# isaac-chandler/cuda-raytracer

Measured on AMD Instinct MI355X. Metric: Mrays/s (live ray segments/s, teapot), higher is better.
Workload: dtype f32

## Files before the change

### cuda-raytracer_amd/csrc/rt_device.h

```cpp
#pragma once
#include <hip/hip_runtime.h>
#include <stdint.h>

#pragma clang fp contract(off)

#define RT_HD __host__ __device__ __forceinline__

namespace rtd {

struct V3 { float x, y, z; };

RT_HD V3 v3(float x, float y, float z) { return {x, y, z}; }
RT_HD V3 operator+(V3 a, V3 b) { return {a.x + b.x, a.y + b.y, a.z + b.z}; }
RT_HD V3 operator-(V3 a, V3 b) { return {a.x - b.x, a.y - b.y, a.z - b.z}; }
RT_HD V3 operator*(V3 a, V3 b) { return {a.x * b.x, a.y * b.y, a.z * b.z}; }
RT_HD V3 operator*(float s, V3 v) { return {s * v.x, s * v.y, s * v.z}; }
RT_HD V3 operator-(V3 v) { return {-v.x, -v.y, -v.z}; }
RT_HD float dot(V3 a, V3 b) { return a.x * b.x + a.y * b.y + a.z * b.z; }
RT_HD V3 cross(V3 a, V3 b) {
    return {a.y * b.z - a.z * b.y, a.z * b.x - a.x * b.z, a.x * b.y - a.y * b.x};
}
RT_HD float magsq(V3 v) { return v.x * v.x + v.y * v.y + v.z * v.z; }
RT_HD V3 normalise(V3 v) { return (1.0f / sqrtf(magsq(v))) * v; }
RT_HD float clamp01(float x) { return fmaxf(fminf(x, 1.0f), 0.0f); }
// ... 64 lines not shown
    const V3 a = (o - min_coord) * inv_dim;
    const V3 b = 0.5f * (d + v3(1, 1, 1));
    return (quant_bit(a.z) << 5) | (quant_bit(a.y) << 4) | (quant_bit(a.x) << 3) |
           (quant_bit(b.z) << 2) | (quant_bit(b.y) << 1) | quant_bit(b.x);
}

RT_HD bool slab(float lx, float ly, float lz, float hx, float hy, float hz, V3 o, float ix, float iy, float iz,
                float tmax, float &tmin) {
    tmin = 0.0f;
    float t1 = (lx - o.x) * ix, t2 = (hx - o.x) * ix;
    tmin = fminf(fmaxf(t1, tmin), fmaxf(t2, tmin));
    tmax = fmaxf(fminf(t1, tmax), fminf(t2, tmax));
    t1 = (ly - o.y) * iy; t2 = (hy - o.y) * iy;
    tmin = fminf(fmaxf(t1, tmin), fmaxf(t2, tmin));
    tmax = fmaxf(fminf(t1, tmax), fminf(t2, tmax));
    t1 = (lz - o.z) * iz; t2 = (hz - o.z) * iz;
    tmin = fminf(fmaxf(t1, tmin), fmaxf(t2, tmin));
    tmax = fmaxf(fminf(t1, tmax), fminf(t2, tmax));
    return tmin <= tmax;
}

RT_HD bool ray_triangle(V3 o, V3 d, V3 p1, V3 e1, V3 e2, float closest, float &t) {
    const V3 h = cross(d, e2);
    const float a = dot(h, e1);
    if (a == 0) return false;
    const float f = 1 / a;
    const V3 s = o - p1;
    const float u = dot(s, h) * f;
    if (u < 0 || u > 1) return false;
    const V3 q = cross(s, e1);
    const float v = dot(d, q) * f;
    if (v < 0 || u + v > 1) return false;
    t = dot(e2, q) * f;
    return !(t < kEps || t >= closest);
}

RT_HD bool ray_sphere(V3 o, V3 d, V3 c, float radius, float closest, float &t) {
    const V3 off = c - o;
    const float mhb = dot(off, d);
    const float qc = magsq(off) - radius * radius;
    const float qd = mhb * mhb - qc;
    if (qd < 0) return false;
    const float hs = sqrtf(qd);
    t = mhb - hs;
    if (t < closest && !(t < kEps)) return true;
    t = mhb + hs;
    return t < closest && !(t < kEps);
}

RT_HD V3 sky_color(const float *env, int env_w, int env_h, V3 dir) {
    const float dx = (float)((double)dir.x * -0.386527 + (double)dir.z * 0.922278);
    const float dy = (float)((double)dir.x * -0.922278 + (double)dir.z * -0.386527);
    const float dz = dir.y;
    const float x = fabsf(dx), y = fabsf(dy), z = fabsf(dz);
    const float r = sqrtf(1 - fminf(z, 1.0f));
    const float a = fmaxf(x, y);
    float b = fminf(x, y);
    b = a == 0 ? 0 : b / a;
    float phi = (float)((2 / 3.14159265358979323846) * (double)rt_atan01(b));
    if (x < y) phi = 1 - phi;
    float v = phi * r;
    float u = r - v;
    if (dz < 0) {
        const float old_v = v;
        v = 1 - u;
        u = 1 - old_v;
    }
    u = copysignf(u, dx);
    v = copysignf(v, dy);
    const float cu = (u + 1) * 0.5f, cv = (v + 1) * 0.5f;
    const int tx = (int)((double)(clamp01(cu) * (env_w - 1)) + 0.5);
    const int ty = (int)((double)(clamp01(cv) * (env_h - 1)) + 0.5);
    const float *e = env + (size_t)(ty * env_h + tx) * 3;
    return v3(e[0], e[1], e[2]);
}

struct Mat { V3 diffuse; float metal; V3 spec; float rough; V3 emit; float ior; };

RT_HD Mat load_mat(const float4 *m) {
    const float4 a = m[0], b = m[1], c = m[2];
    return {v3(a.x, a.y, a.z), a.w, v3(b.x, b.y, b.z), b.w, v3(c.x, c.y, c.z), c.w};
}

RT_HD void scatter(V3 d, V3 normal, const Mat &m, Rng &rng, V3 &T, V3 &C, V3 &nd) {
    C = C + m.emit * T;
    const bool front = dot(normal, d) < 0;
    if (!front) normal = -normal;
    const V3 rough = normalise(normal + m.rough * random_on_sphere(rng));
    const float cos_theta = dot(rough, d);
    if (m.ior == 0) {
        if (random01(rng) <= m.metal) {
            T = T * m.spec;
            nd = d - (2 * cos_theta) * rough;
        } else {
            T = T * m.diffuse;
            nd = normalise(normal + random_on_sphere(rng));
        }
    } else {
        float ior = m.ior;
        float inv_ior = 1 / ior;
        if (front) { const float tmp = inv_ior; inv_ior = ior; ior = tmp; }
        const float sin2 = 1 - cos_theta * cos_theta;
        float r0 = (1 - ior) / (1 + ior);
        r0 *= r0;
        const float cs = 1 + cos_theta;
        const float refl = r0 + (1 - r0) * cs * cs * cs * cs * cs;
        if (sin2 > inv_ior * inv_ior || random01(rng) < refl) {
            T = T * m.spec;
            nd = d - (2 * cos_theta) * rough;
        } else {
            T = T * m.diffuse;
            const V3 perp = ior * (d - cos_theta * rough);
            const V3 par = (-sqrtf(1 - magsq(perp))) * rough;
            nd = normalise(par + perp);
        }
    }
}

}
```

### cuda-raytracer_amd/csrc/rt_render.hip

```cpp
#include "rt_common.h"

#include <algorithm>
#include <chrono>
#include <cstdio>
#include <cstdlib>
#include <cstring>
#include <string>
#include <thread>
#include <vector>

#include <rccl/rccl.h>

#pragma clang fp contract(off)

int rtamd_render_multi(const rt_scene *scene, const rt_opts *opts, float *fb_out, rt_stats *stats);

using namespace rtamd;

namespace {

#ifndef RT_INFLIGHT
#define RT_INFLIGHT 20
#endif
#ifndef RT_TRACE_OCC
// ... 169 lines not shown
            const bool empty = sp == 0;
            sp = empty ? 0 : sp - 1;
            uint2 e = col[min(sp, kStackLds) * kBlock];
            asm volatile("" : "+v"(e.x), "+v"(e.y));
            if (__builtin_expect(__ballot(sp >= kStackLds) != 0, 0)) {
                if (sp >= kStackLds) {
                    e.x = overflow[(sp - kStackLds) * lanes + gl];
                    e.y = overflow[dist_half + (sp - kStackLds) * lanes + gl];
                }
            }
            const bool take = !empty && !(__uint_as_float(e.y) >= closest);
            slot = empty ? -2 - slot : slot;
            ref = take ? e.x : ref;
            if (COUNT) pn += take ? 1u : 0u;
            const bool leaf = take && (ref & kLeaf);
            if (__builtin_expect(leaf && (ref & kBigLeaf), 0)) {
                leaf_range(S, ref, ti, te);
            } else {
                ti = leaf ? (int)(ref & 0xFFFFFFu) : ti;
                te = leaf ? ti + (int)((ref >> 24) & 0x3Fu) : te;
            }
            need = !empty && (!take || (leaf && ti == te));
        }
    };
    const bool root_internal = !(S.root_ref & kLeaf);
    float4 ra{0, 0, 0, 0}, rb{0, 0, 0, 0}, rc{0, 0, 0, 0};
    uint2 rk{0, 0};
    if (root_internal) {
        const float4 *rr = S.nodes + (size_t)S.root_ref * 4;
        const float4 x0 = rr[0], x1 = rr[1], x2 = rr[2];
        const uint2 k = *reinterpret_cast<const uint2 *>(rr + 3);
#define RT_U(v) __int_as_float(__builtin_amdgcn_readfirstlane(__float_as_int(v)))
        ra = make_float4(RT_U(x0.x), RT_U(x0.y), RT_U(x0.z), RT_U(x0.w));
        rb = make_float4(RT_U(x1.x), RT_U(x1.y), RT_U(x1.z), RT_U(x1.w));
        rc = make_float4(RT_U(x2.x), RT_U(x2.y), RT_U(x2.z), RT_U(x2.w));
#undef RT_U
        rk = make_uint2(__builtin_amdgcn_readfirstlane(k.x), __builtin_amdgcn_readfirstlane(k.y));
    }
    while (true) {
        unsigned long long idle = __ballot(slot < 0);
        if (!exhausted && __popcll(idle) >= (FIRST ? kRefillFirst : kRefill)) {
            PROF(6, 1);
            if (slot <= -2) {
                hits[-2 - slot] = make_float2(closest, __int_as_float(index));
                slot = -1;
            }
            bool fresh = false;
            do {
                bool got = false;
                while (idle && !exhausted) {
                    if (q_next >= q_end) {
                        const uint32_t seg_lo = (uint32_t)(((uint64_t)L * shard) / kQueues);
                        const uint32_t seg_hi = (uint32_t)(((uint64_t)L * (shard + 1)) / kQueues);
                        uint32_t c = 0;
                        if (lane_id() == 0) c = atomicAdd(queue + shard * kQueueStride, chunk);
                        c = __builtin_amdgcn_readfirstlane(__shfl(c, 0)) + seg_lo;
                        if (c >= seg_hi) {
                            shard = (shard + 1) % kQueues;
                            if (++tried == kQueues) exhausted = true;
                            continue;
                        }
                        q_next = c;
                        q_end = min(c + chunk, seg_hi);
                    }
                    const uint32_t avail = q_end - q_next;
                    const uint32_t r = rank_below(idle);
                    const bool take = slot < 0 && r < avail;
                    const unsigned long long took = __ballot(take);
                    if (take) { slot = (int)(q_next + r); fresh = true; got = true; }
                    q_next += (uint32_t)__popcll(took);
                    idle &= ~took;
                }
                if (VSLOT) {
                    if (got && slot_bkt[slot] == kDead) { slot = -1; fresh = false; }
                    idle = __ballot(slot < 0);
                }
            } while (VSLOT && idle && !exhausted);
            if (fresh) {
                {
                    nlive++;
                    if (FIRST) {
                        o = S.cam;
                        d = primary_dir(S, (int)first_ray<FIRST>(pa.map, (uint32_t)slot), pa);
                    } else {
                        const float4 *rp = geo + (size_t)slot * 2;
                        const float4 r0 = rp[0];
                        const float2 r1 = *reinterpret_cast<const float2 *>(rp + 1);
                        o = v3(r0.x, r0.y, r0.z);
                        d = v3(r0.w, r1.x, r1.y);
                    }
                    ix = 1 / d.x; iy = 1 / d.y; iz = 1 / d.z;
                    finite_inv = __builtin_isfinite(ix) && __builtin_isfinite(iy) && __builtin_isfinite(iz);

                    closest = 1e30f;
                    index = -1;
                    for (int i = 0; i < S.sphere_count; i++) {
                        const float4 sph = S.spheres[i];
                        float t;
                        if (ray_sphere(o, d, v3(sph.x, sph.y, sph.z), sph.w, closest, t)) { closest = t; index = i; }
                    }
                    ref = S.root_ref;
                    sp = 0;
                    if (COUNT) pn++;
                    ti = te = 0;
                    if (ref & kLeaf) {
                        leaf_range(S, ref, ti, te);
                        if (ti == te) {
                            hits[slot] = make_float2(closest, __int_as_float(index));
                            slot = -1;
                        }
                    }
                }
            }
            wave_nonfinite = __ballot(slot >= 0 && !finite_inv) != 0;
            if (root_internal && __ballot(fresh && slot >= 0)) {
                bool need = false;
                if (fresh && slot >= 0) need = node_step(ra, rb, rc, rk);
                pop_loop(need);
            }
        }
        if (!__ballot(slot >= 0)) {
            if (exhausted) break;
            PROF(7, 1);
            continue;
        }
#ifdef RT_PROFILE
        {
            const unsigned long long act = __ballot(slot >= 0), lf = __ballot(slot >= 0 && ti < te);
            PROF(0, 1); PROF(1, __popcll(act)); PROF(2, __popcll(lf));
            PROF(3, lf != 0); PROF(4, (act & ~lf) != 0);
            const bool mixed = lf != 0 && (act & ~lf) != 0;
            PROF(8, mixed);
            if (mixed) PROF(9, min(__popcll(lf), __popcll(act & ~lf)));
            const uintptr_t ra = slot >= 0 ? (uintptr_t)(ti < te ? S.tris + (size_t)ti * 3 : S.nodes + (size_t)ref * 4) : 0;
            const int first = __builtin_ctzll(act);
            const uintptr_t r0 = ((uintptr_t)__shfl((unsigned)(ra >> 32), first) << 32) | __shfl((unsigned)ra, first);
            const unsigned long long same = __ballot(slot >= 0 && ra == r0);
            PROF(12, same == act);
            PROF(13, 4 * __popcll(same) >= 3 * __popcll(act));
        }
#endif
        if (slot < 0) continue;
        bool need = false;
        const bool in_leaf = ti < te;
        const float4 *rec = in_leaf ? S.tris + (size_t)ti * 3 : S.nodes + (size_t)ref * 4;
        const float4 a = rec[0], b = rec[1], c = rec[2];
        uint2 kids = make_uint2(0, 0);
        if (!in_leaf) kids = *reinterpret_cast<const uint2 *>(rec + 3);
        if (in_leaf) {
            const float4 q0 = a, q1 = b;
            const float q2 = c.x;
            if (COUNT) tt++;
            float t;
            const bool hit =
                ray_triangle_flat(o, d, v3(q0.x, q0.y, q0.z), v3(q0.w, q1.x, q1.y), v3(q1.z, q1.w, q2), closest, t);
            closest = hit ? t : closest;
            index = hit ? S.sphere_count + ti : index;
            need = ++ti == te;
        } else {
            need = node_step(a, b, c, kids);
        }
#ifdef RT_PROFILE
        if (__ballot(need)) PROF(5, 1);
#endif
        pop_loop(need);
    }
    if (slot <= -2) hits[-2 - slot] = make_float2(closest, __int_as_float(index));
    Counters *cs = ctr + ((blockIdx.x * (kBlock / 64) + (threadIdx.x >> 6)) & (kCtrSlots - 1));
    const unsigned long long nl = wave_sum(nlive);
    if (COUNT) {
        const unsigned long long a = wave_sum(pn), b = wave_sum(iv), t = wave_sum(tt);
        if (lane_id() == 0) {
            atomicAdd(&cs->pn, a);
            atomicAdd(&cs->iv, b);
            atomicAdd(&cs->tt, t);
            atomicAdd(&cs->st, nl * (unsigned long long)S.sphere_count);
        }
    }
    if (lane_id() == 0 && nl) atomicAdd(&cs->live, nl);
    if (tspan) {
        __syncthreads();
        if (threadIdx.x == 0) {
            atomicMin(&tspan[blockIdx.x % kSpanSlots], t_start);
            atomicMax(&tspan[kSpanSlots + blockIdx.x % kSpanSlots], (unsigned long long)wall_clock64());
        }
    }
#ifdef RT_PROFILE
    prof[11] = wave_sum((unsigned)prof[10]);
    if (lane_id() == 0)
        for (int i = 0; i < 14; i++)
            if (i != 10) atomicAdd(&g_prof[FIRST ? 0 : 1][i], prof[i]);
#endif
}

struct Shaded {
    V3 no, nd, T;
    V3 C;
    uint32_t ray;
    int kind;
    bool acc_holds;
};
struct ShadeIn {
    float2 h;
    uint32_t ray, seed;
    bool acc_holds;
    float4 r0, r1;
    float tz;
};
template <bool SORTED, int FIRST, bool INLINE>
__device__ __forceinline__ ShadeIn shade_in(const PassArgs &pa, int slot, const float4 *__restrict__ geo,
                                            const float *__restrict__ tz, const uint32_t *__restrict__ rid,
                                            const float2 *__restrict__ hits, const uint32_t *__restrict__ seed_of) {
    ShadeIn in{};
    const uint32_t ray0 = first_ray<FIRST>(pa.map, (uint32_t)slot);
    const uint32_t rv = FIRST ? (FIRST == 2 ? ray0 : (uint32_t)slot) : rid[slot];
    in.ray = rv & ~kAccFlag;
    in.acc_holds = (rv & kAccFlag) != 0;
    in.seed = (!FIRST && seed_of) ? seed_of[slot] : (SORTED || FIRST) ? (FIRST == 2 ? ray0 : (uint32_t)slot) : in.ray;
    if (!INLINE) in.h = hits[slot];
    if (!FIRST) {
        in.r0 = geo[(size_t)slot * 2];
        in.r1 = geo[(size_t)slot * 2 + 1];
        in.tz = tz[slot];
    }
    return in;
}
template <bool SORTED, int FIRST, bool INLINE = false>
__device__ __forceinline__ Shaded shade_from(const DevScene &S, const PassArgs &pa, int slot, const ShadeIn &in,
                                             uint32_t seed_term) {
    Rng rng = pcg_seed(in.seed * 4137874753u + seed_term);
    float closest = in.h.x;
    int index = __float_as_int(in.h.y);
    const uint32_t ray_id = in.ray;
    V3 o, d, T;
    V3 C = v3(0, 0, 0);
    if (FIRST) {
        o = S.cam;
        d = primary_dir(S, (int)(FIRST == 2 ? in.ray : (uint32_t)slot), pa);
        float tx = 1.f, ty = 1.f, tz = 1.f;
        asm volatile("" : "+v"(tx), "+v"(ty), "+v"(tz));
        T = v3(tx, ty, tz);
    } else {
        o = v3(in.r0.x, in.r0.y, in.r0.z);
        d = v3(in.r0.w, in.r1.x, in.r1.y);
        T = v3(in.r1.z, in.r1.w, in.tz);
    }
    if (INLINE) {
        closest = 1e30f;
        index = -1;
        for (int i = 0; i < S.sphere_count; i++) {
            const float4 sph = S.spheres[i];
            float t;
            if (ray_sphere(o, d, v3(sph.x, sph.y, sph.z), sph.w, closest, t)) { closest = t; index = i; }
        }
    }
    V3 no = o, nd = d;
    if (index == -1) {
        C = C + sky_color(S.env, S.env_w, S.env_h, d) * T;
        T = v3(0, 0, 0);
    } else {
        const bool sphere = index < S.sphere_count;
        const uint32_t mi = S.mat_idx[index];
        float4 q = *(sphere ? S.spheres + index : S.tris + (size_t)(index - S.sphere_count) * 3 + 2);
        asm volatile("" : "+v"(q.x), "+v"(q.y), "+v"(q.z), "+v"(q.w));
        no = o + closest * d;
        const V3 normal = sphere ? (1 / q.w) * (no - v3(q.x, q.y, q.z)) : v3(q.y, q.z, q.w);
        const float4 *mp = S.mats + (size_t)mi * 3;
        float4 m0 = mp[0], m1 = mp[1], m2 = mp[2];
        asm volatile("" : "+v"(m0.x), "+v"(m0.y), "+v"(m0.z), "+v"(m0.w), "+v"(m1.x), "+v"(m1.y), "+v"(m1.z),
                          "+v"(m1.w), "+v"(m2.x), "+v"(m2.y), "+v"(m2.z), "+v"(m2.w));
        const Mat m{v3(m0.x, m0.y, m0.z), m0.w, v3(m1.x, m1.y, m1.z), m1.w, v3(m2.x, m2.y, m2.z), m2.w};
        scatter(d, normal, m, rng, T, C, nd);
    }
    return Shaded{no, nd, T, C, ray_id, index == -1 ? 0 : (index < S.sphere_count ? 2 : 1), in.acc_holds};
}
template <bool SORTED, int FIRST, bool INLINE = false>
__device__ __forceinline__ Shaded shade_one(const DevScene &S, const PassArgs &pa, int slot,
                                            const float4 *__restrict__ geo, const float *__restrict__ tz,
                                            const uint32_t *__restrict__ rid, const float2 *__restrict__ hits,
                                            uint32_t seed_term, const uint32_t *__restrict__ seed_of = nullptr) {
    return shade_from<SORTED, FIRST, INLINE>(S, pa, slot, shade_in<SORTED, FIRST, INLINE>(pa, slot, geo, tz, rid, hits, seed_of),
                                             seed_term);
}
__device__ __forceinline__ bool has_radiance(V3 c) {
    return ((__float_as_uint(c.x) | __float_as_uint(c.y) | __float_as_uint(c.z)) & 0x7fffffffu) != 0;
}

__device__ __forceinline__ unsigned long long match_bucket(uint32_t b, bool valid);

#ifndef RT_SHADE_WPE
#define RT_SHADE_WPE 8
#endif
#ifndef RT_REPLAY_WPE
#define RT_REPLAY_WPE 8
#endif
#if RT_REPLAY_WPE > 0
#define RT_REPLAY_ATTR __attribute__((amdgpu_waves_per_eu(RT_REPLAY_WPE, RT_REPLAY_WPE)))
#else
#define RT_REPLAY_ATTR
#endif
#if RT_SHADE_WPE > 0
#define RT_SHADE_ATTR __attribute__((amdgpu_waves_per_eu(RT_SHADE_WPE, RT_SHADE_WPE)))
#else
#define RT_SHADE_ATTR
#endif
template <bool SORTED, bool COUNT, int FIRST, bool FUSED, bool INLINE>
__global__ __launch_bounds__(kBlock) RT_SHADE_ATTR void shade_kernel(DevScene S, PassArgs pa, float4 *__restrict__ geo,
                                                       float *__restrict__ tz, uint32_t *__restrict__ rid,
                                                       float4 *__restrict__ acc, uint8_t *__restrict__ bkt,
                                                       const uint32_t *__restrict__ live_count,
                                                       const float2 *__restrict__ hits, uint32_t seed_term, int last,
                                                       Counters *__restrict__ ctr,
                                                       const uint32_t *__restrict__ seed_of = nullptr,
                                                       uint32_t *__restrict__ counts = nullptr, int tiles = 0,
                                                       int home = 0) {
    const int L = (int)__builtin_amdgcn_readfirstlane(*live_count);
    unsigned hit = 0, miss = 0, hit_sphere = 0;
    auto shade_slot = [&](int slot) -> uint32_t {
        const Shaded sh = shade_one<SORTED, FIRST, INLINE>(S, pa, slot, geo, tz, rid, hits, seed_term, seed_of);
        const V3 no = sh.no, nd = sh.nd, T = sh.T;
        miss += sh.kind == 0;
        hit += sh.kind != 0;
        hit_sphere += sh.kind == 2;
        const bool dead = is_black(T);
        if (!FUSED && !dead && !last) {
            geo[(size_t)slot * 2] = make_float4(no.x, no.y, no.z, nd.x);
            geo[(size_t)slot * 2 + 1] = make_float4(nd.y, nd.z, T.x, T.y);
            tz[slot] = T.z;
        }
        const bool term = has_radiance(sh.C);
        if (dead || last || (term && !(FIRST && home))) {
            V3 C = sh.C;
            const uint32_t dst = sh.ray;
            if (sh.acc_holds) {
                const float4 a = acc[dst];
                C = v3(a.y, a.z, a.w) + sh.C;
            }
            typedef float f4v __attribute__((ext_vector_type(4)));
            if (dead || last)
                __builtin_nontemporal_store(f4v{T.z, C.x, C.y, C.z}, reinterpret_cast<f4v *>(acc + dst));
            else
                acc[dst] = make_float4(T.z, C.x, C.y, C.z);
        }
        if (!FUSED && !dead && !last && (FIRST || (term && !sh.acc_holds)))
            rid[slot] = sh.ray | (term || sh.acc_holds ? kAccFlag : 0u);
        const uint32_t bk = dead ? kDead : (SORTED ? bucket_of(no, nd, S.min_coord, S.inv_dim) : 0u);
        if (!last) bkt[slot] = (uint8_t)bk;
        return bk;
    };
    if (counts && !last) {
        __shared__ uint32_t h[kBuckets];
        const int R = tile_rounds(L), span = kBlock * R;
        for (int tile = blockIdx.x; tile * span < L; tile += gridDim.x) {
            for (int b = threadIdx.x; b < kBuckets; b += kBlock) h[b] = 0;
            __syncthreads();
            const int base = tile * span;
            const int rounds = min(R, (L - base + kBlock - 1) / kBlock);
            for (int r = 0; r < rounds; r++) {
                const int slot = base + r * kBlock + threadIdx.x;
                const bool valid = slot < L;
                const uint32_t bk = valid ? shade_slot(slot) : 0u;
                const unsigned long long peers = match_bucket(bk, valid);
                if (valid && rank_below(peers) == 0) atomicAdd(&h[bk], (uint32_t)__popcll(peers));
            }
            __syncthreads();
            for (int b = threadIdx.x; b < kBuckets; b += kBlock) counts[(size_t)b * tiles + tile] = h[b];
            __syncthreads();
        }
    } else {
        for (int base = blockIdx.x * kBlock; base < L; base += gridDim.x * kBlock) {
            const int slot = base + threadIdx.x;
            if (slot < L) (void)shade_slot(slot);
        }
    }
    if (INLINE) {
        Counters *cs = ctr + ((blockIdx.x * (kBlock / 64) + (threadIdx.x >> 6)) & (kCtrSlots - 1));
        const unsigned long long nl = wave_sum(hit + miss);
        if (lane_id() == 0 && nl) {
            atomicAdd(&cs->live, nl);
            if (COUNT) {
                atomicAdd(&cs->pn, nl);
                atomicAdd(&cs->st, nl * (unsigned long long)S.sphere_count);
            }
        }
    }
    if (COUNT) {
        Counters *cs = ctr + ((blockIdx.x * (kBlock / 64) + (threadIdx.x >> 6)) & (kCtrSlots - 1));
        const unsigned long long h = wave_sum(hit), m = wave_sum(miss), hs = wave_sum(hit_sphere);
        if (lane_id() == 0 && (h | m)) {
            atomicAdd(&cs->hits, h);
            atomicAdd(&cs->misses, m);
            atomicAdd(&cs->hits_sphere, hs);
        }
    }
}

__global__ void fill_live_kernel(uint32_t *__restrict__ live, uint32_t n, int count, uint32_t *__restrict__ queue,
                                 unsigned long long *__restrict__ tspan) {
    const int i = blockIdx.x * blockDim.x + threadIdx.x;
    if (i < count) live[i] = n;
    for (int k = i; k < count * kQueues * kQueueStride; k += blockDim.x) queue[k] = 0;
    if (tspan)
        for (int k = i; k < kSpanWords * count; k += blockDim.x) tspan[k] = (k % kSpanWords) >= kSpanSlots ? 0ull : ~0ull;
}


__device__ __forceinline__ unsigned long long match_bucket(uint32_t b, bool valid) {
    unsigned long long peers = __ballot(valid);
#pragma unroll
    for (int bit = 0; bit < 7; bit++) {
        const unsigned long long m = __ballot((b >> bit) & 1u);
        peers &= ((b >> bit) & 1u) ? m : ~m;
    }
    return peers;
}

__device__ __forceinline__ void bucket_runs(uint32_t *run, const uint32_t *__restrict__ offsets,
                                            const uint32_t *__restrict__ totals, int tiles, int tile) {
    static_assert(kBuckets == 65 && kDead == 64, "buckets 0..63 in one wave, the terminated bucket after them");
    if (threadIdx.x < 64) {
        const int b = (int)threadIdx.x;
        const uint32_t t = totals[b];
        uint32_t x = t;
#pragma unroll
        for (int off = 1; off < 64; off <<= 1) {
            const uint32_t y = __shfl_up(x, off);
            if (b >= off) x += y;
        }
        run[b] = x - t + offsets[(size_t)b * tiles + tile];
        if (b == 63) run[kDead] = x + offsets[(size_t)kDead * tiles + tile];
// ... 243 lines not shown
__global__ void set_count_kernel(uint32_t *__restrict__ dst, uint32_t v, const uint32_t *__restrict__ src) {
    if (threadIdx.x == 0) *dst = src ? *src : v;
}

template <bool SORTED, int FIRST, bool INLINE>
__global__ __launch_bounds__(kBlock) RT_REPLAY_ATTR void sort_scatter_shade_kernel(DevScene S, PassArgs pa,
                                                                    const uint8_t *__restrict__ bkt_in,
                                                                    const float4 *__restrict__ geo_in,
                                                                    const float *__restrict__ tz_in,
                                                                    const uint32_t *__restrict__ rid_in,
                                                                    const float2 *__restrict__ hits, uint32_t seed_term,
                                                                    const uint32_t *__restrict__ live_count, int tiles,
                                                                    const uint32_t *__restrict__ offsets,
                                                                    const uint32_t *__restrict__ totals,
                                                                    float4 *__restrict__ geo_out,
                                                                    float *__restrict__ tz_out,
                                                                    uint32_t *__restrict__ rid_out,
                                                                    float4 *__restrict__ acc = nullptr,
                                                                    uint32_t *__restrict__ home_of = nullptr,
                                                                    uint32_t home_base = 0) {
    const bool homes = FIRST == 1 && home_of != nullptr;
    const int n = (int)*live_count;
    __shared__ uint32_t run[kBuckets];
    __shared__ uint32_t wcount[kBlock / 64][kBuckets];
    const int R = tile_rounds(n), span = kBlock * R;
    for (int tile = blockIdx.x; tile * span < n; tile += gridDim.x) {
        bucket_runs(run, offsets, totals, tiles, tile);
        for (int k = threadIdx.x; k < (kBlock / 64) * kBuckets; k += kBlock) (&wcount[0][0])[k] = 0;
        __syncthreads();
        const int wave = threadIdx.x >> 6;
        const int base = tile * span;
        const int rounds = min(R, (n - base + kBlock - 1) / kBlock);
        for (int r = 0; r < rounds; r++) {
            const int item = base + r * kBlock + threadIdx.x;
            const bool valid = item < n;
            const uint32_t b = valid ? bkt_in[item] : 0u;
            const bool move = valid && b != kDead;
            Shaded sh{};
            if (move) sh = shade_one<SORTED, FIRST, INLINE>(S, pa, item, geo_in, tz_in, rid_in, hits, seed_term);
            const unsigned long long peers = match_bucket(b, valid);
            const uint32_t rank = rank_below(peers);
            if (valid && rank == 0) wcount[wave][b] = (uint32_t)__popcll(peers);
            __syncthreads();
            if (move) {
                uint32_t pos = run[b] + rank;
                for (int k = 0; k < wave; k++) pos += wcount[k][b];
                geo_out[(size_t)pos * 2] = make_float4(sh.no.x, sh.no.y, sh.no.z, sh.nd.x);
                geo_out[(size_t)pos * 2 + 1] = make_float4(sh.nd.y, sh.nd.z, sh.T.x, sh.T.y);
                tz_out[pos] = sh.T.z;
                const uint32_t id = homes ? home_base + pos : sh.ray;
                if (homes) {
                    home_of[item] = id;
                    if (has_radiance(sh.C)) acc[id] = make_float4(sh.T.z, sh.C.x, sh.C.y, sh.C.z);
                }
                rid_out[pos] = id | (has_radiance(sh.C) || sh.acc_holds ? kAccFlag : 0u);
            } else if (homes && valid) {
                home_of[item] = (uint32_t)item;
            }
            __syncthreads();
            if (threadIdx.x < kBuckets) {
                uint32_t s = 0;
                for (int k = 0; k < kBlock / 64; k++) { s += wcount[k][threadIdx.x]; wcount[k][threadIdx.x] = 0; }
                run[threadIdx.x] += s;
            }
            __syncthreads();
        }
    }
}


__global__ __launch_bounds__(kBlock) void fill_dead_kernel(uint8_t *__restrict__ bkt, const uint32_t *__restrict__ count) {
    const uint32_t n = *count;
    const uint32_t n16 = n / 16;
    const uint32_t w = kDead * 0x01010101u;
    for (uint32_t i = blockIdx.x * kBlock + threadIdx.x; i < n16; i += gridDim.x * kBlock)
        reinterpret_cast<uint4 *>(bkt)[i] = make_uint4(w, w, w, w);
    for (uint32_t i = n16 * 16 + blockIdx.x * kBlock + threadIdx.x; i < n; i += gridDim.x * kBlock) bkt[i] = (uint8_t)kDead;
}

template <bool COUNT>
__global__ __launch_bounds__(kBlock) RT_SHADE_ATTR void shade_rank_kernel(DevScene S, PassArgs pa,
                                                            const uint8_t *__restrict__ bkt_in,
                                                            const float4 *__restrict__ geo_in,
                                                            const float *__restrict__ tz_in,
                                                            const uint32_t *__restrict__ rid_in,
                                                            const float2 *__restrict__ hits, uint32_t seed_term, int last,
                                                            const uint32_t *__restrict__ slot_count, int tiles,
                                                            const uint32_t *__restrict__ offsets,
                                                            const uint32_t *__restrict__ totals,
                                                            float4 *__restrict__ geo_out, float *__restrict__ tz_out,
                                                            uint32_t *__restrict__ rid_out, uint8_t *__restrict__ bkt_out,
                                                            float4 *__restrict__ acc, Counters *__restrict__ ctr) {
    const int n = (int)__builtin_amdgcn_readfirstlane(*slot_count);
    __shared__ uint32_t run[kBuckets];
    __shared__ uint32_t wcount[kBlock / 64][kBuckets];
    unsigned hit = 0, miss = 0, hit_sphere = 0;
    const int R = tile_rounds(n), span = kBlock * R;
    for (int tile = blockIdx.x; tile * span < n; tile += gridDim.x) {
        bucket_runs(run, offsets, totals, tiles, tile);
        for (int k = threadIdx.x; k < (kBlock / 64) * kBuckets; k += kBlock) (&wcount[0][0])[k] = 0;
        __syncthreads();
        const int wave = threadIdx.x >> 6;
        const int base = tile * span;
        const int rounds = min(R, (n - base + kBlock - 1) / kBlock);
        for (int r = 0; r < rounds; r++) {
            const int item = base + r * kBlock + threadIdx.x;
            const bool valid = item < n;
            const uint32_t b = valid ? bkt_in[item] : 0u;
            const bool move = valid && b != kDead;
            ShadeIn in{};
            if (move) in = shade_in<true, 0, false>(pa, item, geo_in, tz_in, rid_in, hits, nullptr);
            const unsigned long long peers = match_bucket(b, valid);
            const uint32_t rank = rank_below(peers);
            if (valid && rank == 0) wcount[wave][b] = (uint32_t)__popcll(peers);
            __syncthreads();
            if (move) {
                uint32_t pos = run[b] + rank;
                for (int k = 0; k < wave; k++) pos += wcount[k][b];
                in.seed = pos;
                const Shaded sh = shade_from<true, 0>(S, pa, item, in, seed_term);
                const V3 no = sh.no, nd = sh.nd, T = sh.T;
                miss += sh.kind == 0;
                hit += sh.kind != 0;
                hit_sphere += sh.kind == 2;
                const bool dead = is_black(T);
                const bool term = has_radiance(sh.C);
                if (dead || last || term) {
                    V3 C = sh.C;
                    if (sh.acc_holds) {
                        const float4 a = acc[sh.ray];
                        C = v3(a.y, a.z, a.w) + sh.C;
                    }
                    typedef float f4v __attribute__((ext_vector_type(4)));
                    if (dead || last)
                        __builtin_nontemporal_store(f4v{T.z, C.x, C.y, C.z}, reinterpret_cast<f4v *>(acc + sh.ray));
                    else
                        acc[sh.ray] = make_float4(T.z, C.x, C.y, C.z);
                }
                if (!dead && !last) {
                    geo_out[(size_t)pos * 2] = make_float4(no.x, no.y, no.z, nd.x);
                    geo_out[(size_t)pos * 2 + 1] = make_float4(nd.y, nd.z, T.x, T.y);
                    tz_out[pos] = T.z;
                    rid_out[pos] = sh.ray | (term || sh.acc_holds ? kAccFlag : 0u);
                    bkt_out[pos] = (uint8_t)bucket_of(no, nd, S.min_coord, S.inv_dim);
                }
            }
            __syncthreads();
            if (threadIdx.x < kBuckets) {
                uint32_t s = 0;
                for (int k = 0; k < kBlock / 64; k++) { s += wcount[k][threadIdx.x]; wcount[k][threadIdx.x] = 0; }
                run[threadIdx.x] += s;
            }
            __syncthreads();
        }
    }
    if (COUNT) {
        Counters *cs = ctr + ((blockIdx.x * (kBlock / 64) + (threadIdx.x >> 6)) & (kCtrSlots - 1));
        const unsigned long long h = wave_sum(hit), m = wave_sum(miss), hs = wave_sum(hit_sphere);
        if (lane_id() == 0 && (h | m)) {
            atomicAdd(&cs->hits, h);
            atomicAdd(&cs->misses, m);
            atomicAdd(&cs->hits_sphere, hs);
        }
    }
}

constexpr int kAccPixels = 64;
template <bool TILED>
__global__ __launch_bounds__(kBlock) void accumulate_kernel(const float4 *__restrict__ tc, int rtc, int pixels,
                                                            float *__restrict__ sums, SlotMap pix,
                                                            const uint32_t *__restrict__ home_of = nullptr) {
    __shared__ float col[kAccPixels * 20 * 3];
    const int p0 = blockIdx.x * kAccPixels;
    const int np = min(kAccPixels, pixels - p0);
    const int n = np * rtc;
    const float4 *src = tc + (size_t)p0 * rtc;
    for (int e = threadIdx.x; e < n; e += kBlock) {
        const float4 c = TILED     ? tc[(size_t)pix.ray((uint32_t)(p0 + e / rtc)) * rtc + e % rtc]
                         : home_of ? tc[home_of[(size_t)p0 * rtc + e]]
                                   : src[e];
        col[e * 3] = c.y;
        col[e * 3 + 1] = c.z;
        col[e * 3 + 2] = c.w;
    }
    __syncthreads();
    const int t = threadIdx.x;
    if (t >= np) return;
    float sx = 0, sy = 0, sz = 0;
    const float *r = col + t * rtc * 3;
    for (int s = 0; s < rtc; s++) {
        sx = sx + r[s * 3];
        sy = sy + r[s * 3 + 1];
        sz = sz + r[s * 3 + 2];
    }
    const size_t p = TILED ? (size_t)pix.ray((uint32_t)(p0 + t)) : (size_t)(p0 + t);
    sums[p * 3] = sx;
    sums[p * 3 + 1] = sy;
    sums[p * 3 + 2] = sz;
}

__global__ __launch_bounds__(kBlock) void high_pass_kernel(const float *__restrict__ img, float *__restrict__ out,
// ... 271 lines not shown
                                             " passes in flight; set RTAMD_INFLIGHT to the same lower value on every owner");
        const int inflight = nctx;
        for (int k = 0; k < inflight; k++) {
            PassCtx &c = ctx[k];
            if ((rc = c.open())) return rc;
            for (int q = 0; q < 2; q++) {
                if ((rc = c.geo[q].alloc((size_t)max_rays * 2))) return rc;
                if ((rc = c.tz[q].alloc((size_t)max_rays))) return rc;
                if ((rc = c.rid[q].alloc((size_t)max_rays))) return rc;
            }
            if ((rc = c.bkt.alloc((size_t)max_rays))) return rc;
            if (vre && (rc = c.bkt1.alloc((size_t)max_rays))) return rc;
            if ((rc = c.acc.alloc((size_t)max_rays * (home ? 2 : 1)))) return rc;
            if (home && (rc = c.home_of.alloc((size_t)max_rays))) return rc;
            if ((rc = c.sort_counts.alloc((size_t)kBuckets * tiles))) return rc;
            if ((rc = c.sort_offsets.alloc((size_t)kBuckets * tiles))) return rc;
            if ((rc = c.sort_totals.alloc(kBuckets))) return rc;
            if ((rc = c.live.alloc((size_t)bounces + 1))) return rc;
            if ((rc = c.queue.alloc((size_t)(bounces + 1) * kQueues * kQueueStride))) return rc;
            if ((rc = c.hits.alloc((size_t)max_rays))) return rc;
            if ((rc = c.overflow.alloc((size_t)trace_blocks_max * kBlock * 2 * (kStackMax - kStackLds)))) return rc;
            if ((rc = c.psum.alloc((size_t)pixels * 3))) return rc;
            if (tsort()) {
                for (int q = 0; q < 2; q++)
                    if ((rc = c.gslot[q].alloc((size_t)max_rays))) return rc;
                if ((rc = c.newpos.alloc((size_t)max_rays)) || (rc = c.gbytes.alloc((size_t)max_rays)) ||
                    (rc = c.lbytes.alloc((size_t)max_rays)) || (rc = c.glive.alloc(3)))
                    return rc;
                HIPCHK(hipHostMalloc(reinterpret_cast<void **>(&c.lg_host), sizeof(uint32_t)));
                HIPCHK(hipEventCreateWithFlags(&c.lg_ready, hipEventDisableTiming));
            }
        }
        tm.mark("pass contexts");
        HIPCHK(hipMemsetAsync(fb.p, 0, fb.n * sizeof(float), s0));
        HIPCHK(hipStreamSynchronize(s0));
        tm.mark("sync");
        if (tm.on) tm.out += vre ? " bounce-0 reorder: virtual" : " bounce-0 reorder: moved";
        tm.report();
        return RT_OK;
    }

    int enqueue_pass(PassCtx &c, int p, float *sums, int64_t &sorted, unsigned long long *tspan) {
        const int before = spp - 20 * p;
        const int rtc = std::min(before, 20);
        const int remaining = before - rtc;
        const int64_t pixels = (int64_t)width * height;
        const int64_t tpix = tile_pixels();
        const int n = (int)(rtc * tpix);
        const int grid = blocks_for(n);
        const int tiles = tile_stride(n);
        const int tgrid = std::min(grid, trace_blocks);
        const int sgrid = std::min(grid, scene.cus * RT_SHADE_BPC);
        const int sort_grid = std::max(1, std::min(max_tiles(n), RT_SORT_GRID > 0 ? RT_SORT_GRID : scene.cus * 8));
        hipStream_t st = c.stream;
        int cur = 0;
        if (n == 0) {
            for (int k = 0; pass_events && k < 3 * bounces + 2 * (bounces - 1); k++) {
                hipEvent_t e = c.event();
                if (!e) return rtamd::fail(RT_E_HIP, "hipEventCreate failed");
                HIPCHK(hipEventRecord(e, st));
            }
            HIPCHK(hipMemsetAsync(sums, 0, (size_t)pixels * 3 * sizeof(float), st));
            return RT_OK;
        }
        hipLaunchKernelGGL(fill_live_kernel, dim3(1), dim3(256), 0, st, c.live.p, (uint32_t)n, bounces + 1, c.queue.p, tspan);
        const uint32_t stripe_px = (uint32_t)(tile_rows * width);
        const SlotMap pix = tiled() ? SlotMap::of(stripe_px, tile_count, tile_index) : SlotMap::identity();
        const SlotMap map = tiled() ? SlotMap::of(stripe_px * (uint32_t)rtc, tile_count, tile_index) : SlotMap::identity();
        const PassArgs pa{rtc, 709579u * (uint32_t)remaining, FastDiv::of((uint32_t)rtc), FastDiv::of((uint32_t)width),
                          map};
        for (int b = 0; b < bounces; b++) {
            const uint32_t seed_term = 279220567u * (uint32_t)(remaining * 20 + b);
            hipEvent_t e0 = nullptr, em = nullptr, e1 = nullptr;
            if (pass_events) {
                e0 = c.event(); em = c.event(); e1 = c.event();
                if (!e0 || !em || !e1) return rtamd::fail(RT_E_HIP, "hipEventCreate failed");
                HIPCHK(hipEventRecord(e0, st));
            }
            const uint32_t *lv = c.live.p + b;
            uint32_t *q = c.queue.p + (size_t)b * kQueues * kQueueStride;
            const bool last = b + 1 == bounces;
            const bool v0 = vre && b == 0, v1 = vre && b == 1;
            const bool fuse_b = !v0 && !v1 && (fused || b <= fused_upto);
            uint32_t *hist = shade_hist && !last && !v1 ? c.sort_counts.p : nullptr;
#define RT_PROCESS3(SORTED, COUNT, FIRST)                                                                        \
    do {                                                                                                         \
        if (!inline_hits)                                                                                        \
            hipLaunchKernelGGL((trace_kernel<SORTED, COUNT, FIRST>), dim3(tgrid), dim3(kBlock), 0, st, scene.ds, pa, \
                               c.geo[cur].p, lv, q, c.hits.p, c.overflow.p, scene.ctr.p,                         \
                               tspan ? tspan + kSpanWords * b : nullptr);                                        \
        if (em) HIPCHK(hipEventRecord(em, st));                                                                  \
        if (inline_hits)                                                                                         \
            hipLaunchKernelGGL((shade_kernel<SORTED, COUNT, FIRST, true, true>), dim3(sgrid), dim3(kBlock), 0, st,\
                               scene.ds, pa, c.geo[cur].p, c.tz[cur].p, c.rid[cur].p, c.acc.p, c.bkt.p, lv, c.hits.p, \
                               seed_term, (int)last, scene.ctr.p, nullptr, hist, tiles, (int)(home && b == 0));  \
        else if (fuse_b)                                                                                         \
            hipLaunchKernelGGL((shade_kernel<SORTED, COUNT, FIRST, true, false>), dim3(sgrid), dim3(kBlock), 0, \
                               st, scene.ds, pa, c.geo[cur].p, c.tz[cur].p, c.rid[cur].p, c.acc.p, c.bkt.p, lv, c.hits.p, \
                               seed_term, (int)last, scene.ctr.p, nullptr, hist, tiles, (int)(home && b == 0));  \
        else                                                                                                     \
            hipLaunchKernelGGL((shade_kernel<SORTED, COUNT, FIRST, false, false>), dim3(sgrid), dim3(kBlock), 0, \
                               st, scene.ds, pa, c.geo[cur].p, c.tz[cur].p, c.rid[cur].p, c.acc.p, c.bkt.p, lv, c.hits.p, \
                               seed_term, (int)last, scene.ctr.p, nullptr, hist, tiles, (int)(home && b == 0));  \
    } while (0)
#define RT_PROCESS(SORTED, COUNT)                                                                                \
    do {                                                                                                         \
        if (b == 0) RT_PROCESS3(SORTED, COUNT, 1); else RT_PROCESS3(SORTED, COUNT, 0);                           \
    } while (0)
            if (v1) {
#define RT_VPROCESS(COUNT)                                                                                       \
    do {                                                                                                         \
        hipLaunchKernelGGL((trace_kernel<true, COUNT, 0, true>), dim3(tgrid), dim3(kBlock), 0, st, scene.ds, pa, \
                           c.geo[cur].p, c.live.p, q, c.hits.p, c.overflow.p, scene.ctr.p,                       \
                           tspan ? tspan + kSpanWords * b : nullptr, c.bkt.p);                                   \
        if (em) HIPCHK(hipEventRecord(em, st));                                                                  \
        hipLaunchKernelGGL((shade_rank_kernel<COUNT>), dim3(sort_grid), dim3(kBlock), 0, st, scene.ds, pa, c.bkt.p, \
                           c.geo[cur].p, c.tz[cur].p, c.rid[cur].p, c.hits.p, seed_term, (int)last, c.live.p, tiles, \
                           c.sort_offsets.p, c.sort_totals.p, c.geo[1 - cur].p, c.tz[1 - cur].p, c.rid[1 - cur].p, \
                           c.bkt1.p, c.acc.p, scene.ctr.p);                                                      \
    } while (0)
                if (counters) RT_VPROCESS(true); else RT_VPROCESS(false);
#undef RT_VPROCESS
                cur = 1 - cur;
            } else if (sort) {
                if (counters) RT_PROCESS(true, true); else RT_PROCESS(true, false);
            } else {
                if (b == 0 && tiled()) {
                    if (counters) RT_PROCESS3(false, true, 2); else RT_PROCESS3(false, false, 2);
                } else if (counters) RT_PROCESS(false, true); else RT_PROCESS(false, false);
            }
#undef RT_PROCESS
#undef RT_PROCESS3
            HIPCHK(hipGetLastError());
            if (pass_events) HIPCHK(hipEventRecord(e1, st));
            if (b + 1 != bounces) {
                hipEvent_t s0 = nullptr, s1 = nullptr;
                if (pass_events) {
                    s0 = c.event(); s1 = c.event();
                    if (!s0 || !s1) return rtamd::fail(RT_E_HIP, "hipEventCreate failed");
                    HIPCHK(hipEventRecord(s0, st));
                }
                const uint8_t *bk = v1 ? c.bkt1.p : c.bkt.p;
                if (!hist)
                    hipLaunchKernelGGL(sort_hist_kernel, dim3(sort_grid), dim3(kBlock), 0, st, bk, lv, tiles,
                                       c.sort_counts.p);
                hipLaunchKernelGGL(sort_scan_kernel, dim3(kBuckets), dim3(kBlock), 0, st, c.sort_counts.p, lv, tiles,
                                   c.sort_offsets.p, c.sort_totals.p, c.live.p + b + 1);
                if (v0) {
                    if (b + 2 != bounces)
                        hipLaunchKernelGGL(fill_dead_kernel, dim3(sort_grid), dim3(kBlock), 0, st, c.bkt1.p, c.live.p + 1);
                } else if (fuse_b) {
#define RT_FSC2(SO, FI, IN)                                                                                      \
    hipLaunchKernelGGL((sort_scatter_shade_kernel<SO, FI, IN>), dim3(sort_grid), dim3(kBlock), 0, st, scene.ds, pa, \
                       c.bkt.p, c.geo[cur].p, c.tz[cur].p, c.rid[cur].p, c.hits.p, seed_term, lv, tiles,          \
                       c.sort_offsets.p, c.sort_totals.p, c.geo[1 - cur].p, c.tz[1 - cur].p, c.rid[1 - cur].p,    \
                       c.acc.p, home && b == 0 ? c.home_of.p : nullptr, home_base)
#define RT_FSC(SO, FI) do { if (inline_hits) RT_FSC2(SO, FI, true); else RT_FSC2(SO, FI, false); } while (0)
                    if (sort) {
                        if (b == 0) RT_FSC(true, 1); else RT_FSC(true, 0);
                    } else {
                        if (b == 0 && tiled()) RT_FSC(false, 2); else if (b == 0) RT_FSC(false, 1); else RT_FSC(false, 0);
                    }
#undef RT_FSC
#undef RT_FSC2
                } else if (b == 0 && tiled())
                    hipLaunchKernelGGL(sort_scatter_kernel<2>, dim3(sort_grid), dim3(kBlock), 0, st, c.bkt.p, c.geo[cur].p,
                                       c.tz[cur].p, c.rid[cur].p, lv, tiles, c.sort_offsets.p, c.sort_totals.p,
                                       c.geo[1 - cur].p, c.tz[1 - cur].p, c.rid[1 - cur].p, pa.map);
                else if (b == 0)
                    hipLaunchKernelGGL(sort_scatter_kernel<1>, dim3(sort_grid), dim3(kBlock), 0, st, c.bkt.p, c.geo[cur].p,
                                       c.tz[cur].p, c.rid[cur].p, lv, tiles, c.sort_offsets.p, c.sort_totals.p,
                                       c.geo[1 - cur].p, c.tz[1 - cur].p, c.rid[1 - cur].p, pa.map);
                else
                    hipLaunchKernelGGL(sort_scatter_kernel<0>, dim3(sort_grid), dim3(kBlock), 0, st, bk, c.geo[cur].p,
                                       c.tz[cur].p, c.rid[cur].p, lv, tiles, c.sort_offsets.p, c.sort_totals.p,
                                       c.geo[1 - cur].p, c.tz[1 - cur].p, c.rid[1 - cur].p, pa.map);
                HIPCHK(hipGetLastError());
                if (pass_events) HIPCHK(hipEventRecord(s1, st));
                if (!v0) cur = 1 - cur;
                if (sort) sorted += n;
            }
        }
        if (bounces == 0) {
            HIPCHK(hipMemsetAsync(sums, 0, (size_t)pixels * 3 * sizeof(float), st));
        } else if (!tiled()) {
            hipLaunchKernelGGL(accumulate_kernel<false>, dim3((unsigned)((pixels + kAccPixels - 1) / kAccPixels)),
                               dim3(kBlock), 0, st, c.acc.p, rtc, (int)pixels, sums, pix, home ? c.home_of.p : nullptr);
        } else {
            HIPCHK(hipMemsetAsync(sums, 0, (size_t)pixels * 3 * sizeof(float), st));
            if (tpix > 0)
                hipLaunchKernelGGL(accumulate_kernel<true>, dim3((unsigned)((tpix + kAccPixels - 1) / kAccPixels)),
                                   dim3(kBlock), 0, st, c.acc.p, rtc, (int)tpix, sums, pix);
        }
        HIPCHK(hipGetLastError());
        return RT_OK;
    }

    int wait_event(hipEvent_t e) {
        if (!xpoll) {
            HIPCHK(hipEventSynchronize(e));
            return RT_OK;
        }
// ... 774 lines not shown
```

Measured before the change: 14300.

## Slim bounce-0 ray hand-over: store pos/dir plus material id and spec bit

When the vre path is on, bounce 0 now runs a SLIM shade kernel. It writes only origin and direction as three float2s, a 16-bit material index in the tz buffer, and a spec flag packed into the bucket byte. It no longer writes throughput, the ray id and the accumulator flag. The bounce-1 trace and the shade_rank kernel rebuild throughput and acc_holds from the material table, using the fact that T starts at (1,1,1) on bounce 0. This cuts global memory traffic between the first two bounces, but it adds material lookups and relies on exact reconstruction of T.

```diff
diff --git a/cuda-raytracer_amd/csrc/rt_device.h b/cuda-raytracer_amd/csrc/rt_device.h
--- a/cuda-raytracer_amd/csrc/rt_device.h
+++ b/cuda-raytracer_amd/csrc/rt_device.h
@@ -170,14 +170,16 @@
     return {v3(a.x, a.y, a.z), a.w, v3(b.x, b.y, b.z), b.w, v3(c.x, c.y, c.z), c.w};
 }
 
-RT_HD void scatter(V3 d, V3 normal, const Mat &m, Rng &rng, V3 &T, V3 &C, V3 &nd) {
+RT_HD bool scatter(V3 d, V3 normal, const Mat &m, Rng &rng, V3 &T, V3 &C, V3 &nd) {
+    bool spec;
     C = C + m.emit * T;
     const bool front = dot(normal, d) < 0;
     if (!front) normal = -normal;
     const V3 rough = normalise(normal + m.rough * random_on_sphere(rng));
     const float cos_theta = dot(rough, d);
     if (m.ior == 0) {
-        if (random01(rng) <= m.metal) {
+        spec = random01(rng) <= m.metal;
+        if (spec) {
             T = T * m.spec;
             nd = d - (2 * cos_theta) * rough;
         } else {
@@ -193,7 +195,8 @@
         r0 *= r0;
         const float cs = 1 + cos_theta;
         const float refl = r0 + (1 - r0) * cs * cs * cs * cs * cs;
-        if (sin2 > inv_ior * inv_ior || random01(rng) < refl) {
+        spec = sin2 > inv_ior * inv_ior || random01(rng) < refl;
+        if (spec) {
             T = T * m.spec;
             nd = d - (2 * cos_theta) * rough;
         } else {
@@ -203,6 +206,7 @@
             nd = normalise(par + perp);
         }
     }
-}
-
-}
+    return spec;
+}
+
+}
diff --git a/cuda-raytracer_amd/csrc/rt_render.hip b/cuda-raytracer_amd/csrc/rt_render.hip
--- a/cuda-raytracer_amd/csrc/rt_render.hip
+++ b/cuda-raytracer_amd/csrc/rt_render.hip
@@ -275,6 +275,11 @@
                     if (FIRST) {
                         o = S.cam;
                         d = primary_dir(S, (int)first_ray<FIRST>(pa.map, (uint32_t)slot), pa);
+                    } else if (VSLOT) {
+                        const float2 *rp = reinterpret_cast<const float2 *>(geo) + (size_t)slot * 3;
+                        const float2 r0 = rp[0], r1 = rp[1], r2 = rp[2];
+                        o = v3(r0.x, r0.y, r1.x);
+                        d = v3(r1.y, r2.x, r2.y);
                     } else {
                         const float4 *rp = geo + (size_t)slot * 2;
                         const float4 r0 = rp[0];
@@ -392,7 +397,10 @@
     uint32_t ray;
     int kind;
     bool acc_holds;
+    uint32_t mat;
+    bool spec;
 };
+constexpr uint32_t kSpecBit = 0x80;
 struct ShadeIn {
     float2 h;
     uint32_t ray, seed;
@@ -418,9 +426,12 @@
     }
     return in;
 }
-template <bool SORTED, int FIRST, bool INLINE = false>
+template <bool SORTED, int FIRST, bool INLINE = false, bool SLIM = false>
 __device__ __forceinline__ Shaded shade_from(const DevScene &S, const PassArgs &pa, int slot, const ShadeIn &in,
                                              uint32_t seed_term) {
+    static_assert(!SLIM || FIRST == 1, "the slim hand-over leaves bounce 0, where T enters as (1,1,1)");
+    uint32_t mat = 0;
+    bool spec = false;
     Rng rng = pcg_seed(in.seed * 4137874753u + seed_term);
     float closest = in.h.x;
     int index = __float_as_int(in.h.y);
@@ -463,17 +474,22 @@
         asm volatile("" : "+v"(m0.x), "+v"(m0.y), "+v"(m0.z), "+v"(m0.w), "+v"(m1.x), "+v"(m1.y), "+v"(m1.z),
                           "+v"(m1.w), "+v"(m2.x), "+v"(m2.y), "+v"(m2.z), "+v"(m2.w));
         const Mat m{v3(m0.x, m0.y, m0.z), m0.w, v3(m1.x, m1.y, m1.z), m1.w, v3(m2.x, m2.y, m2.z), m2.w};
-        scatter(d, normal, m, rng, T, C, nd);
-    }
-    return Shaded{no, nd, T, C, ray_id, index == -1 ? 0 : (index < S.sphere_count ? 2 : 1), in.acc_holds};
-}
-template <bool SORTED, int FIRST, bool INLINE = false>
+        const bool took_spec = scatter(d, normal, m, rng, T, C, nd);
+        if (SLIM) {
+            spec = took_spec;
+            mat = mi;
+        }
+    }
+    return Shaded{no, nd, T, C, ray_id, index == -1 ? 0 : (index < S.sphere_count ? 2 : 1), in.acc_holds, mat, spec};
+}
+template <bool SORTED, int FIRST, bool INLINE = false, bool SLIM = false>
 __device__ __forceinline__ Shaded shade_one(const DevScene &S, const PassArgs &pa, int slot,
                                             const float4 *__restrict__ geo, const float *__restrict__ tz,
                                             const uint32_t *__restrict__ rid, const float2 *__restrict__ hits,
                                             uint32_t seed_term, const uint32_t *__restrict__ seed_of = nullptr) {
-    return shade_from<SORTED, FIRST, INLINE>(S, pa, slot, shade_in<SORTED, FIRST, INLINE>(pa, slot, geo, tz, rid, hits, seed_of),
-                                             seed_term);
+    return shade_from<SORTED, FIRST, INLINE, SLIM>(S, pa, slot,
+                                                   shade_in<SORTED, FIRST, INLINE>(pa, slot, geo, tz, rid, hits, seed_of),
+                                                   seed_term);
 }
 __device__ __forceinline__ bool has_radiance(V3 c) {
     return ((__float_as_uint(c.x) | __float_as_uint(c.y) | __float_as_uint(c.z)) & 0x7fffffffu) != 0;
@@ -497,7 +513,7 @@
 #else
 #define RT_SHADE_ATTR
 #endif
-template <bool SORTED, bool COUNT, int FIRST, bool FUSED, bool INLINE>
+template <bool SORTED, bool COUNT, int FIRST, bool FUSED, bool INLINE, bool SLIM = false>
 __global__ __launch_bounds__(kBlock) RT_SHADE_ATTR void shade_kernel(DevScene S, PassArgs pa, float4 *__restrict__ geo,
                                                        float *__restrict__ tz, uint32_t *__restrict__ rid,
                                                        float4 *__restrict__ acc, uint8_t *__restrict__ bkt,
@@ -510,13 +526,20 @@
     const int L = (int)__builtin_amdgcn_readfirstlane(*live_count);
     unsigned hit = 0, miss = 0, hit_sphere = 0;
     auto shade_slot = [&](int slot) -> uint32_t {
-        const Shaded sh = shade_one<SORTED, FIRST, INLINE>(S, pa, slot, geo, tz, rid, hits, seed_term, seed_of);
+        const Shaded sh = shade_one<SORTED, FIRST, INLINE, SLIM>(S, pa, slot, geo, tz, rid, hits, seed_term, seed_of);
         const V3 no = sh.no, nd = sh.nd, T = sh.T;
         miss += sh.kind == 0;
         hit += sh.kind != 0;
         hit_sphere += sh.kind == 2;
         const bool dead = is_black(T);
-        if (!FUSED && !dead && !last) {
+        if (SLIM && !dead && !last) {
+            float2 *rec = reinterpret_cast<float2 *>(geo) + (size_t)slot * 3;
+            rec[0] = make_float2(no.x, no.y);
+            rec[1] = make_float2(no.z, nd.x);
+            rec[2] = make_float2(nd.y, nd.z);
+            reinterpret_cast<uint16_t *>(tz)[slot] = (uint16_t)sh.mat;
+        }
+        if (!SLIM && !FUSED && !dead && !last) {
             geo[(size_t)slot * 2] = make_float4(no.x, no.y, no.z, nd.x);
             geo[(size_t)slot * 2 + 1] = make_float4(nd.y, nd.z, T.x, T.y);
             tz[slot] = T.z;
@@ -535,10 +558,10 @@
             else
                 acc[dst] = make_float4(T.z, C.x, C.y, C.z);
         }
-        if (!FUSED && !dead && !last && (FIRST || (term && !sh.acc_holds)))
+        if (!SLIM && !FUSED && !dead && !last && (FIRST || (term && !sh.acc_holds)))
             rid[slot] = sh.ray | (term || sh.acc_holds ? kAccFlag : 0u);
         const uint32_t bk = dead ? kDead : (SORTED ? bucket_of(no, nd, S.min_coord, S.inv_dim) : 0u);
-        if (!last) bkt[slot] = (uint8_t)bk;
+        if (!last) bkt[slot] = (uint8_t)(bk | (SLIM && !dead && sh.spec ? kSpecBit : 0u));
         return bk;
     };
     if (counts && !last) {
@@ -948,8 +971,7 @@
 __global__ __launch_bounds__(kBlock) RT_SHADE_ATTR void shade_rank_kernel(DevScene S, PassArgs pa,
                                                             const uint8_t *__restrict__ bkt_in,
                                                             const float4 *__restrict__ geo_in,
-                                                            const float *__restrict__ tz_in,
-                                                            const uint32_t *__restrict__ rid_in,
+                                                            const uint16_t *__restrict__ mat_in,
                                                             const float2 *__restrict__ hits, uint32_t seed_term, int last,
                                                             const uint32_t *__restrict__ slot_count, int tiles,
                                                             const uint32_t *__restrict__ offsets,
@@ -972,10 +994,20 @@
         for (int r = 0; r < rounds; r++) {
             const int item = base + r * kBlock + threadIdx.x;
             const bool valid = item < n;
-            const uint32_t b = valid ? bkt_in[item] : 0u;
+            const uint32_t byte = valid ? bkt_in[item] : 0u;
+            const uint32_t b = byte & ~kSpecBit;
             const bool move = valid && b != kDead;
             ShadeIn in{};
-            if (move) in = shade_in<true, 0, false>(pa, item, geo_in, tz_in, rid_in, hits, nullptr);
+            float2 r0{}, r1{}, r2{};
+            float4 alb{}, emi{};
+            if (move) {
+                const float4 *mp = S.mats + (size_t)mat_in[item] * 3;
+                in.h = hits[item];
+                const float2 *rp = reinterpret_cast<const float2 *>(geo_in) + (size_t)item * 3;
+                r0 = rp[0]; r1 = rp[1]; r2 = rp[2];
+                alb = mp[byte & kSpecBit ? 1 : 0];
+                emi = mp[2];
+            }
             const unsigned long long peers = match_bucket(b, valid);
             const uint32_t rank = rank_below(peers);
             if (valid && rank == 0) wcount[wave][b] = (uint32_t)__popcll(peers);
@@ -983,6 +1015,15 @@
             if (move) {
                 uint32_t pos = run[b] + rank;
                 for (int k = 0; k < wave; k++) pos += wcount[k][b];
+                float one = 1.f;
+                asm volatile("" : "+v"(one));
+                const V3 ones = v3(one, one, one);
+                const V3 T0 = ones * v3(alb.x, alb.y, alb.z);
+                in.r0 = make_float4(r0.x, r0.y, r1.x, r1.y);
+                in.r1 = make_float4(r2.x, r2.y, T0.x, T0.y);
+                in.tz = T0.z;
+                in.ray = (uint32_t)item;
+                in.acc_holds = has_radiance(v3(0, 0, 0) + v3(emi.x, emi.y, emi.z) * ones);
                 in.seed = pos;
                 const Shaded sh = shade_from<true, 0>(S, pa, item, in, seed_term);
                 const V3 no = sh.no, nd = sh.nd, T = sh.T;
@@ -1420,7 +1461,7 @@
             const bool last = b + 1 == bounces;
             const bool v0 = vre && b == 0, v1 = vre && b == 1;
             const bool fuse_b = !v0 && !v1 && (fused || b <= fused_upto);
-            uint32_t *hist = shade_hist && !last && !v1 ? c.sort_counts.p : nullptr;
+            uint32_t *hist = (shade_hist || v0) && !last && !v1 ? c.sort_counts.p : nullptr;
 #define RT_PROCESS3(SORTED, COUNT, FIRST)                                                                        \
     do {                                                                                                         \
         if (!inline_hits)                                                                                        \
@@ -1445,7 +1486,20 @@
     do {                                                                                                         \
         if (b == 0) RT_PROCESS3(SORTED, COUNT, 1); else RT_PROCESS3(SORTED, COUNT, 0);                           \
     } while (0)
-            if (v1) {
+            if (v0) {
+#define RT_V0PROCESS(COUNT)                                                                                      \
+    do {                                                                                                         \
+        hipLaunchKernelGGL((trace_kernel<true, COUNT, 1>), dim3(tgrid), dim3(kBlock), 0, st, scene.ds, pa,       \
+                           c.geo[cur].p, lv, q, c.hits.p, c.overflow.p, scene.ctr.p,                             \
+                           tspan ? tspan + kSpanWords * b : nullptr);                                            \
+        if (em) HIPCHK(hipEventRecord(em, st));                                                                  \
+        hipLaunchKernelGGL((shade_kernel<true, COUNT, 1, false, false, true>), dim3(sgrid), dim3(kBlock), 0, st, \
+                           scene.ds, pa, c.geo[cur].p, c.tz[cur].p, c.rid[cur].p, c.acc.p, c.bkt.p, lv, c.hits.p, \
+                           seed_term, (int)last, scene.ctr.p, nullptr, hist, tiles, 0);                          \
+    } while (0)
+                if (counters) RT_V0PROCESS(true); else RT_V0PROCESS(false);
+#undef RT_V0PROCESS
+            } else if (v1) {
 #define RT_VPROCESS(COUNT)                                                                                       \
     do {                                                                                                         \
         hipLaunchKernelGGL((trace_kernel<true, COUNT, 0, true>), dim3(tgrid), dim3(kBlock), 0, st, scene.ds, pa, \
@@ -1453,9 +1507,9 @@
                            tspan ? tspan + kSpanWords * b : nullptr, c.bkt.p);                                   \
         if (em) HIPCHK(hipEventRecord(em, st));                                                                  \
         hipLaunchKernelGGL((shade_rank_kernel<COUNT>), dim3(sort_grid), dim3(kBlock), 0, st, scene.ds, pa, c.bkt.p, \
-                           c.geo[cur].p, c.tz[cur].p, c.rid[cur].p, c.hits.p, seed_term, (int)last, c.live.p, tiles, \
-                           c.sort_offsets.p, c.sort_totals.p, c.geo[1 - cur].p, c.tz[1 - cur].p, c.rid[1 - cur].p, \
-                           c.bkt1.p, c.acc.p, scene.ctr.p);                                                      \
+                           c.geo[cur].p, reinterpret_cast<const uint16_t *>(c.tz[cur].p), c.hits.p, seed_term,   \
+                           (int)last, c.live.p, tiles, c.sort_offsets.p, c.sort_totals.p, c.geo[1 - cur].p,      \
+                           c.tz[1 - cur].p, c.rid[1 - cur].p, c.bkt1.p, c.acc.p, scene.ctr.p);                   \
     } while (0)
                 if (counters) RT_VPROCESS(true); else RT_VPROCESS(false);
 #undef RT_VPROCESS
```

After: 14800, median of 6. 1.03x the previous value.
